# raphiniert-com/volume_renderer

Measured on AMD Instinct MI355X. Metric: Mrays/s + achieved HBM GB/s, 1024³ vol @ 1920×1080 HG-shaded, 1/2/4/8 GPU, higher is better.
Workload: dtype f32; 1 GPU; V_shell(1024) fp32 1024^3, 1920x1080, HG 2 lights (example1.m), on-the-fly gradient, rotate(125,25,0) f=3 dist=6 thr=0.9; lights=2, gradient=compute, parallelism=image-column partition x1 (block 16), depth_lanes=2, frames=serial, one HIP stream

## Files before the change

### volume_renderer_amd/csrc/vr_capi.hip

```cpp
#include <hip/hip_runtime.h>

#include <algorithm>
#include <chrono>
#include <cmath>
#include <cstdio>
#include <cstdlib>
#include <cstring>
#include <memory>
#include <mutex>
#include <map>
#include <set>
#include <array>
#include <sstream>
#include <string>
#include <queue>
#include <vector>

#include "../../include/vrhip.h"
#include "vr_device.h"
#include "vr_resources.h"

#ifndef VR_WITH_K8
#define VR_WITH_K8 0
#endif
// ... 661 lines not shown
  F.mode = P.num_lights == 0 ? 0 : (g_tex.grad_method == G_LOOKUP ? 2 : 1);
  F.ab_alias = same_tex(P.ab, P.em);
  const bool em_grid = P.em.p && !P.em.one;
  if (F.mode == 1)
    F.share = em_grid && same_tex(P.gem, P.em);
  else if (F.mode == 2)
    F.share = em_grid && P.gx.p && P.gy.p && P.gz.p && !P.gx.one && same_dims(P.gx, P.em) &&
              same_dims(P.gy, P.em) && same_dims(P.gz, P.em);
  P.re_is_em = same_tex(P.re, P.em) && P.em.p != nullptr;
  {
    drift_bound(F, nullptr);
    for (int i = 0; i < 3; ++i) {
      const float n = i == 0 ? P.em.fnx : (i == 1 ? P.em.fny : P.em.fnz);
      P.tap_off[i] = (float)((F.mode == 1 ? (double)P.gstep[i] * P.bscale[i] * n : 0.0) + 0.0625);
    }
    P.tap_half = half_texel_taps(P, F.mode, P.em.fnz);
    P.cube_hs[0] = P.tap_half ? P.em.fnx * 0.5f : 0.f;
    P.cube_hs[1] = P.tap_half ? P.em.fny * 0.5f : 0.f;
    P.cube_hs[2] = P.tap_half ? P.em.fnz * 0.5f : 0.f;
  }
  {
    const BufPtr &rb = g_tex.bind[g_tex.idx_re];
    const BufPtr &lb = g_tex.bind[T_LIGHT];
    bool ok = tame(rb) && tame(lb) && std::isfinite(P.fr) && std::fabs(P.fr) < 1e3f;
    double bound = 1.0;
    for (int i = 0; i < 3; ++i) {
      ok = ok && std::isfinite(P.color[i]) && std::fabs(P.color[i]) < 1e3f;
      bound = std::max(bound, (double)std::fabs(P.color[i]));
    }
    double lmax = 0.0;
    for (const auto &L : g_tex.lights) {
      for (float c : {L.cr, L.cg, L.cb}) {
        ok = ok && std::isfinite(c);
        lmax = std::max(lmax, (double)std::fabs(c));
      }
    }
    const double rmax = (rb && rb->ptr) ? rb->maxabs : 0.0, lutmax = (lb && lb->ptr) ? lb->maxabs : 0.0;
    ok = ok && (double)std::fabs(P.fr) * rmax * lutmax * lmax * bound * (double)(g_tex.lights.size() + 1) < 1e36;
    P.skip_empty = ok ? 1 : 0;
    if (const char *ev = test_env("VR_NO_EMPTY_SKIP"))
      if (ev[0] == '1') P.skip_empty = 0;
  }
  {
    const BufPtr &eb = g_tex.bind[g_tex.idx_em], &ab = g_tex.bind[g_tex.idx_ab];
    auto vmax = [](const BufPtr &b) { return (b && b->ptr) ? (b->nonfinite ? INFINITY : (double)b->maxabs) : 0.0; };
    const double xa = std::fabs((double)P.fa) * vmax(ab) * (double)P.tstep;
    const double xe = std::fabs((double)P.fe) * vmax(eb) * (double)P.tstep;
    P.small_x = (std::isfinite(xa) && xa < 0x1p-7 * 0.999) ? 1 : 0;
    P.eds_finite = (std::isfinite(xe) && xe < 1e38) ? 1 : 0;
    if (diag_flag("VR_NO_RANGE_FLAGS")) P.small_x = P.eds_finite = 0;
  }
  {
    const bool re_ok = P.re_is_em || (P.re.p && P.re.one);
    const bool lut_ok = g_tex.lights.empty() || (P.lut.p && P.lut.small && !P.lut.one && P.lut.zp);
    const bool step_ok = std::isfinite(P.tstep) && P.tstep > 0.f;
    P.tame = (P.skip_empty && P.eds_finite && P.small_x && re_ok && lut_ok && step_ok && !diag_flag("VR_NO_TAME")) ? 1
                                                                                                            : 0;
    P.re_mask = P.re_is_em ? 0xffffffffu : 0u;
  }
  F.big = is_big(P.em) || is_big(P.ab) || is_big(P.re) || is_big(P.gem) || is_big(P.gx) || is_big(P.gy) ||
          is_big(P.gz) || test_flag("VR_FORCE_BIG");
  if (F.mode == 2 && P.gx.p &&
      vr::interleave3_entries(P.gx.px, P.gx.pxy / P.gx.px, (uint32_t)P.gx.nz + 2u) > 0xFFFFFFFFull)
    F.big = true;
  if (is_big(P.lut)) return fail(VR_ERR_UNSUPPORTED, "illumination volume larger than 2^32 voxels");
  bool finite = std::isfinite(P.tstep) && P.tstep > 0.f;
  for (int i = 0; i < 3; ++i) finite = finite && std::isfinite(P.bmin[i]) && std::isfinite(P.bscale[i]);
  const double diag = std::sqrt(4.0 * ((double)bmax[0] * bmax[0] + (double)bmax[1] * bmax[1] +
                                       (double)bmax[2] * bmax[2]));
  const double cap = 2.0 * diag / (double)P.tstep + 64.0;
  P.max_steps = (finite && cap < 2.0e9) ? (int32_t)cap : 2000000000;
  F.degenerate = !finite;
  return VR_OK;
}

void upload_lights(vr_context *h, const vr_render_args *a) {
  if (a->num_lights < 0 || !a->illumination) return;
  const size_t n = (size_t)a->num_lights;
  g_tex.lights.resize(n);
  for (size_t l = 0; l < n; ++l) {
    const vr_light &L = a->lights[l];
    g_tex.lights[l] = vr::DevLight{L.position[2], L.position[1], L.position[0], L.color[0], L.color[1],
                                   L.color[2]};
  }
  h->vol[T_LIGHT] = make_rec(a->illumination);
  sync_volume_if_changed(h, T_LIGHT, T_LIGHT);
}

using LaunchRec = vr_host::LaunchRec<BufPtr>;
void wait_ready(const BufPtr &b, hipStream_t s) {
  if (b && !vr_host::done(b->ready)) VR_HIP(hipStreamWaitEvent(s, b->ready->e, 0));
}
void bind_reads(LaunchRec &L) {
  for (const BufPtr &b : g_tex.bind)
    if (b) {
      wait_ready(b, L.stream);
      L.reads.push_back(b);
    }
  for (const auto &kv : g_tex.gvec)
    if (kv.second.buf && kv.first == L.device) {
      wait_ready(kv.second.buf, L.stream);
      L.reads.push_back(kv.second.buf);
    }
}
void stage_frame(LaunchRec &L, vr::RenderParams &P, const std::vector<vr::DevLight> &lights) {
  const void *d = nullptr;
  VR_HIP(L.stage(lights.data(), lights.size() * sizeof(vr::DevLight), &d));
// ... 1977 lines not shown
```

### volume_renderer_amd/csrc/vr_march.hip

```cpp
#include <hip/hip_runtime.h>
#include <stdint.h>
#include <math.h>
#include <stdlib.h>
#include <algorithm>
#include <type_traits>

#ifndef VR_MARCH_K
#define VR_MARCH_K 1
#endif
#ifndef VR_MERGED_BOUNDS
#define VR_MERGED_BOUNDS 1
#endif
#ifndef VR_WHOLE_BOX
#define VR_WHOLE_BOX 1
#endif
#ifndef VR_CHECK_WHOLE
#define VR_CHECK_WHOLE 0
#endif
#ifndef VR_LIGHTS_HOIST
#define VR_LIGHTS_HOIST 1
#endif
#ifndef VR_REFL_HOIST
#define VR_REFL_HOIST 1
#endif
// ... 282 lines not shown
#undef iny
#undef inz
}

__device__ __forceinline__ void composite(const RenderParams &P, Ray &R, float r, float gg, float b, float alpha,
                                          float thr, int cap) {
  const float om = 1.f - R.sa;
  R.sr = fmaf(om, r, R.sr);
  R.sg = fmaf(om, gg, R.sg);
  R.sb = fmaf(om, b, R.sb);
  R.sa = fmaf(om, alpha, R.sa);
  ++R.nsteps;
  if (R.sa > thr || R.nsteps >= cap) {
    R.alive = false;
  } else {
    R.t += P.tstep;
    if (R.t > R.tfar) R.alive = false;
    else R.pos = mk(R.pos.x + R.step.x, R.pos.y + R.step.y, R.pos.z + R.step.z);
  }
}

#ifndef VR_GROUP_ANY_DPP
#define VR_GROUP_ANY_DPP 1
#endif
template <int K>
__device__ __forceinline__ bool group_any(bool b) {
  if constexpr ((K == 2 || K == 4) && VR_GROUP_ANY_DPP) {
    int v = b ? 1 : 0;
    v |= __builtin_amdgcn_mov_dpp(v, 0xB1, 0xf, 0xf, true);
    if constexpr (K == 4) v |= __builtin_amdgcn_mov_dpp(v, 0x4E, 0xf, 0xf, true);
    return v != 0;
  } else {
    const uint64_t m = __ballot(b);
    const int base = (int)(__lane_id() & ~(uint32_t)(K - 1));
    return ((m >> base) & ((1ull << K) - 1)) != 0ull;
  }
}

template <int K, int I = 0>
__device__ __forceinline__ int group_max_i(int v, int acc) {
  if constexpr (K == 1 || I == K) {
    return acc;
  } else {
    return group_max_i<K, I + 1>(v, max(acc, __float_as_int(group_lane<K, I>(__int_as_float(v)))));
  }
}

#ifndef VR_ZERO_FILL
#define VR_ZERO_FILL 1
#endif
template <int K, int I, bool ZF = false>
__device__ __forceinline__ void composite_group(const RenderParams &P, Ray &R, float exf, float r, float gg, float b,
                                                float alpha, float thr) {
  if constexpr (I < K) {
    const float ri = group_lane<K, I>(r), gi = group_lane<K, I>(gg), bi = group_lane<K, I>(b),
                ai = group_lane<K, I>(alpha);
    if ((ZF || group_lane<K, I>(exf) != 0.f) && R.alive) {
      const float om = 1.f - R.sa;
      R.sr = fmaf(om, ri, R.sr);
      R.sg = fmaf(om, gi, R.sg);
      R.sb = fmaf(om, bi, R.sb);
      R.sa = fmaf(om, ai, R.sa);
      if (R.sa > thr) R.alive = false;
    }
    composite_group<K, I + 1, ZF>(P, R, exf, r, gg, b, alpha, thr);
  }
}

template <int K, int MODE, bool AB_ALIAS, bool COUNT, bool SHARE2, bool BIG, bool NANCHK, int CAP, bool SLAB = false,
          int NL = 0>
__device__ __forceinline__ void march(const RenderParams &P, float *L, int lane, Ray &R, ChunkStats &C,
                                      uint32_t kk = 0, KParams kp = nullptr, uint32_t gw = 0) {
  static_assert(!COUNT || K == 1 || VR_COUNT_K, "the counter variant is built for K = 1 only (VR_COUNT_K: all K)");
  static_assert(!SLAB || (!COUNT && BIG), "slab mode: no counters, 64-bit addressing");
  const int cap = P.max_steps;
  const float thr = P.thr;
  const float sbz = P.bmin[2], ssz = P.bscale[2];
  auto beyond = [&](float zn) { return R.step.z >= 0.f ? zn >= P.slab_z1 : zn < P.slab_z0; };
  const DevTex &E = P.em;
  const int sub = lane & (K - 1);
  if constexpr (K > 1) {
    R.mine = R.alive;
    leap(P, sub, R.mine, R.nsteps, R.t, R.tfar, R.pos, R.step, cap);
    R.alive = group_any<K>(R.mine);
  }

  int s0 = VR_CHUNK;
  constexpr bool PROBE = VR_PROBE && !NANCHK && AB_ALIAS && !SLAB;
  int ps = VR_PROBE_MIN;
  float rv = 0.f;
  if constexpr (!NANCHK && VR_REFL_HOIST) {
    if (P.tame && P.re.p) rv = voxel0(P.re.p);
    asm volatile("" : "+v"(rv));
  }
  DevLight pre2[2];
  const DevLight *pre = nullptr;
  if constexpr (!NANCHK && VR_LIGHTS_HOIST && MODE != 0 && K > 1 && AB_ALIAS && SHARE2 && !BIG && !SLAB && !COUNT) {
    const bool two = NL == 2 || (NL == 0 && P.num_lights >= 2);
    for (int j = 0; j < 2; ++j) {
      pre2[j] = (two || (NL == 1 && j == 0)) ? light_at(P, j) : DevLight{0.f, 0.f, 0.f, 0.f, 0.f, 0.f};
      asm volatile("" : "+v"(pre2[j].px), "+v"(pre2[j].py), "+v"(pre2[j].pz), "+v"(pre2[j].cr), "+v"(pre2[j].cg),
                   "+v"(pre2[j].cb));
    }
    if (two || NL == 1) pre = pre2;
  }
  auto leap_run = [&](int n) __attribute__((always_inline)) {
    if constexpr (K == 1) {
// ... 110 lines not shown
    if (staged) {
      const bool nonzero = stage_box<BIG>(L, E, B, lane);
      empty = AB_ALIAS && P.skip_empty && !partial && !nonzero && (!SLAB || inside);
    }
    __builtin_amdgcn_wave_barrier();
    if (COUNT) ++(staged && !partial ? (empty ? C.leap : C.staged) : C.fall);
    const bool whole = __builtin_amdgcn_readfirstlane((!NANCHK && !SLAB && staged && !partial && !edge) ? 1 : 0) != 0;

    if (empty) {
      if (!parked_any) leap_run(S);
      else if (__float_as_int(R.t) >= 0) leap_run(S);
      unpark();
      if (PROBE && ps < 0) ps = VR_PROBE_MIN;
      continue;
    }
    if (PROBE) ps = (VR_PROBE_LANES && VR_REPROBE_PARTIAL && partial) ? (int)VR_PROBE_MIN : -1;

    if constexpr (K == 1) {
      for (int k = 0; k < S && R.alive; ++k) {
        if (SLAB && !inside) {
          const float zn = (R.pos.z - sbz) * ssz;
          if (!(zn >= P.slab_z0 && zn < P.slab_z1)) {
            if (beyond(zn)) {
              store_resume(P, kk, R.t, R.pos, R.nsteps);
              R.alive = false;
              R.past = true;
            } else {
              ++R.nsteps;
              if (R.nsteps >= P.max_steps) {
                R.alive = false;
              } else {
                R.t += P.tstep;
                if (R.t > R.tfar) R.alive = false;
                else R.pos = mk(R.pos.x + R.step.x, R.pos.y + R.step.y, R.pos.z + R.step.z);
              }
            }
            continue;
          }
        }
        float r, gg, b, alpha;
        bool shaded;
        sample_at<MODE, AB_ALIAS, SHARE2, BIG, NANCHK, NL>(P, L, B, staged, whole, R.pos, R.o, r, gg, b, alpha, shaded,
                                                       rv, pre);
        if (COUNT) {
          ++C.iter;
          C.lit += (MODE != 0 && __any(shaded)) ? 1u : 0u;
          R.nlit += shaded ? 1 : 0;
        }
        composite(P, R, r, gg, b, alpha, thr, cap);
      }
    } else {
      auto samples = [&](auto wc) {
      constexpr bool WC = decltype(wc)::value;
      for (int k = 0; k < S && R.alive; k += K) {
        float r = 0.f, gg = 0.f, b = 0.f, alpha = 0.f;
        bool ex = R.mine, take = R.mine;
        if (SLAB && !inside) {
          const float zn = (R.pos.z - sbz) * ssz;
          if (ex && beyond(zn)) ex = false;
          take = ex && zn >= P.slab_z0 && zn < P.slab_z1;
        }
        bool shaded = false;
        if (take) {
          sample_at<MODE, AB_ALIAS, SHARE2, BIG, NANCHK, NL>(P, L, B, staged, WC || (!VR_WHOLE_SPLIT && whole), R.pos,
                                                         R.o, r, gg, b, alpha, shaded, rv, pre);
        }
        if (COUNT) {
          ++C.iter;
          C.lit += (MODE != 0 && __any(shaded)) ? 1u : 0u;
        }
        composite_group<K, 0, VR_ZERO_FILL && !NANCHK && !SLAB>(P, R, ex ? 1.f : 0.f, r, gg, b, alpha, thr);
        if (SLAB && !inside) {
          if (R.alive && group_any<K>(R.mine && !ex)) {
            float t = R.t;
            f3 p = R.pos;
            int32_t n = R.nsteps;
            first_of_group<K>((R.mine && !ex) ? 1.f : 0.f, R.t, R.pos, R.nsteps, t, p, n);
            if (sub == 0) store_resume(P, kk, t, p, n);
            R.alive = false;
            R.past = true;
          }
        }
        if constexpr (!NANCHK && !SLAB)
          advance_k<K>(P, R.mine, R.nsteps, R.t, R.tfar, R.pos, R.step, cap);
        else
          advance(P, K, R.mine, R.nsteps, R.t, R.tfar, R.pos, R.step, cap);
        R.alive = R.alive && group_any<K>(R.mine);
      }
      };
      if constexpr (VR_WHOLE_SPLIT && !NANCHK && !SLAB && VR_MARCH_FAST && MODE == 1 && SHARE2) {
        if (whole) samples(std::true_type{});
        else samples(std::false_type{});
      } else {
        samples(std::false_type{});
      }
    }
    unpark();
    __builtin_amdgcn_wave_barrier();
  }
}

__device__ __forceinline__ bool finite3(const f3 &v) {
  return fabsf(v.x) <= 3.4e38f && fabsf(v.y) <= 3.4e38f && fabsf(v.z) <= 3.4e38f;
}

#ifndef VR_MARCH_MIN_EU
#define VR_MARCH_MIN_EU 5
// ... 42 lines not shown
    wgo += P.block_rot;
    if (wgo >= gridDim.x) wgo -= gridDim.x;
  }
  if (ORDERED && blockIdx.x < P.prio_blocks) __builtin_amdgcn_s_setprio(2);
  int view, lc, y;
  if constexpr (PAIRED) {
    constexpr int TH2 = TS::TH / 2, HR = (64 / K) / 2;
    const int tile = (int)wgo * VR_WG_WAVES + wave;
    const int nbx = (P.part_cols + P.pair_shift + 2 * TS::TW - 1) / (2 * TS::TW);
    const int blk = tile >> 2, quad = tile & 3;
    const int ray = lane >> TS::LK, rr = ray & (HR - 1);
    view = ray >= HR ? 0 : 1;
    const int xv = (blk % nbx) * (2 * TS::TW) + (quad & 1) * TS::TW + rr / TH2;
    y = (blk / nbx) * (2 * TH2) + (quad >> 1) * TH2 + rr % TH2;
    lc = view ? xv - P.pair_shift : xv;
  } else {
    view = (P.views > 1 && wgo >= P.view_blocks) ? 1 : 0;
    const uint32_t wg = view ? wgo - P.view_blocks : wgo;
    const int tile = (int)wg * VR_WG_WAVES + wave;
    const int nbx = (P.part_cols + 2 * TS::TW - 1) / (2 * TS::TW);
    const int blk = tile >> 2, quad = tile & 3;
    const int ray = lane >> TS::LK;
    lc = (blk % nbx) * (2 * TS::TW) + (quad & 1) * TS::TW + (ray / TS::TH);
    y = (blk / nbx) * (2 * TS::TH) + (quad >> 1) * TS::TH + (ray % TS::TH);
  }
  float *const out = view ? P.out2 : P.out;
  const bool active = (!PAIRED || lc >= 0) && (lc < P.part_cols) && (y < P.height);
  Ray R;
  R.o = mk(0.f, 0.f, 0.f);
  R.pos = R.o;
  R.step = R.o;
  R.t = 0.f;
  R.tfar = -1.f;
  R.sr = R.sg = R.sb = R.sa = 0.f;
  R.nsteps = R.nlit = 0;
  R.alive = false;
  ChunkStats C{0, 0, 0, 0, 0, 0, 0};
  if (active) {
    const int blk = lc / P.block_cols, within = lc - blk * P.block_cols;
    const int x = (P.part + blk * P.num_parts) * P.block_cols + within;
    f3 d;
    float tnear;
    R.alive = ray_setup(P, x, y, R.o, d, tnear, R.tfar, view);
    R.pos = mk(fmaf(d.x, tnear, R.o.x), fmaf(d.y, tnear, R.o.y), fmaf(d.z, tnear, R.o.z));
    R.step = mk(d.x * P.tstep, d.y * P.tstep, d.z * P.tstep);
    R.t = tnear;
  }
  if (P.tame && __all(!R.alive || (finite3(R.pos) && finite3(R.step))))
    march<K, MODE, AB_ALIAS, COUNT, SHARE2, BIG, false, CAP, false, NL>(
        P, L, lane, R, C, 0u, (KParams)__builtin_amdgcn_kernarg_segment_ptr(), wgo * VR_WG_WAVES + (uint32_t)wave);
  else
    march<K, MODE, AB_ALIAS, COUNT, SHARE2, BIG, true, CAP>(P, L, lane, R, C);

  if (active && (lane & (K - 1)) == 0) {
    const size_t plane = (size_t)P.plane_cols * (size_t)P.height;
    const size_t kk = (size_t)lc * (size_t)P.height + (size_t)y;
    out[kk] = R.sr;
    out[kk + plane] = R.sg;
    out[kk + 2 * plane] = R.sb;
  }
  if (TIMED) {
    __syncthreads();
    if (threadIdx.x == 0) {
      const uint64_t d = __builtin_amdgcn_s_memrealtime() - clk0;
      P.wg_cost[wgo] = d > 0xffffffffull ? 0xffffffffu : (uint32_t)d;
      if (P.wg_start) P.wg_start[wgo] = (uint32_t)clk0;
    }
  }
  if (COUNT) {
    unsigned long long s = K == 1 ? (unsigned long long)R.nsteps : 0ull, l = K == 1 ? (unsigned long long)R.nlit : 0ull;
#pragma unroll
    for (int off = 32; off > 0; off >>= 1) {
      s += __shfl_xor(s, off, 64);
      l += __shfl_xor(l, off, 64);
    }
    if (lane == 0 && s) atomicAdd(P.steps, s);
    if (lane == 0 && l) atomicAdd(P.steps + 1, l);
    if (lane == 0) {
      atomicAdd(P.steps + 2, (unsigned long long)C.staged);
      atomicAdd(P.steps + 3, (unsigned long long)C.leap);
      atomicAdd(P.steps + 4, (unsigned long long)C.fall);
      atomicAdd(P.steps + 5, (unsigned long long)C.iter);
      atomicAdd(P.steps + 6, (unsigned long long)C.lit);
      atomicAdd(P.steps + 7, (unsigned long long)C.probe);
      atomicAdd(P.steps + 44, (unsigned long long)C.probe_fail);
    }
  }
}

template <int K>
__global__ __launch_bounds__(64 * VR_WG_WAVES) void preleap_kernel(const RenderParams P) {
  using TS = TileShape<K>;
  const int lane = threadIdx.x & 63, wave = threadIdx.x >> 6;
  const uint32_t wgo = blockIdx.x;
  const uint32_t gw = wgo * VR_WG_WAVES + (uint32_t)wave;
  const int view = (P.views > 1 && wgo >= P.view_blocks) ? 1 : 0;
  const uint32_t wg = view ? wgo - P.view_blocks : wgo;
  const int tile = (int)wg * VR_WG_WAVES + wave;
  const int nbx = (P.part_cols + 2 * TS::TW - 1) / (2 * TS::TW);
  const int blk = tile >> 2, quad = tile & 3;
  const int ray = lane >> TS::LK;
  const int lc = (blk % nbx) * (2 * TS::TW) + (quad & 1) * TS::TW + (ray / TS::TH);
  const int y = (blk / nbx) * (2 * TS::TH) + (quad >> 1) * TS::TH + (ray % TS::TH);
  const bool active = lc < P.part_cols && y < P.height;
  Ray R;
  R.pos = mk(0.f, 0.f, 0.f);
  R.step = R.pos;
// ... 422 lines not shown
```

### volume_renderer_amd/csrc/vr_sampling.h

```cpp
#pragma once
#include <hip/hip_runtime.h>
#include <stdint.h>
#include <math.h>

#include "vr_device.h"

namespace vr {

#define VR_PI ((float)3.14159265358979323846f)

struct f3 {
  float x, y, z;
};
__device__ __forceinline__ f3 mk(float x, float y, float z) { return f3{x, y, z}; }
__device__ __forceinline__ float dot3(f3 a, f3 b) { return fmaf(a.z, b.z, fmaf(a.y, b.y, a.x * b.x)); }

typedef float f2a4 __attribute__((ext_vector_type(2), aligned(4)));
typedef float f4a8 __attribute__((ext_vector_type(4), aligned(8)));

struct Ax {
  int i;
  float w;
};
__device__ __forceinline__ float weight8(float xb, float fl) {
  return fmaf(rintf(xb * 256.f), 1.f / 256.f, -fl);
}
template <bool NANCHK = true>
__device__ __forceinline__ Ax axis(float c, int n, float fn) {
  if (NANCHK) c = (c != c) ? 0.f : c;
  const float xb = c * fn - 0.5f;
  const float fl = floorf(xb);
  const float w = weight8(xb, fl);
  (void)n;
  return Ax{(int)__builtin_amdgcn_fmed3f(fl, -1.f, fn - 1.f), w};
}

template <bool NANCHK = true>
__device__ __forceinline__ Ax axis_raw(float c, float fn) {
  if (NANCHK) c = (c != c) ? 0.f : c;
  const float xb = c * fn - 0.5f;
  const float fl = floorf(xb);
  const float w = weight8(xb, fl);
  return Ax{(int)fl, w};
}
__device__ __forceinline__ Ax clamp_ax(const Ax &a, int n) { return Ax{min(max(a.i, -1), n - 1), a.w}; }

struct AxS {
  int i;
  float w;
  bool hi;
};
template <bool NANCHK = true>
__device__ __forceinline__ AxS axis_raw_s(float c, float fn) {
  if (NANCHK) c = (c != c) ? 0.f : c;
  const float xb = c * fn - 0.5f;
  const float fl = floorf(xb);
  const float r = xb - fl;
  const float w = rintf(r * 256.f) * (1.f / 256.f);
  return AxS{(int)fl, w, r >= 0.5f};
}
template <bool NANCHK = true>
__device__ __forceinline__ AxS axis_cube_s(float p, float hs) {
  float a = p + 1.f;
  if (NANCHK) a = (a != a) ? 0.f : a;
  const float xb = fmaf(a, hs, -0.5f);
  const float fl = floorf(xb);
  const float r = xb - fl;
  const float w = rintf(r * 256.f) * (1.f / 256.f);
  return AxS{(int)fl, w, r >= 0.5f};
}

__device__ __forceinline__ void half_taps(const AxS &a, Ax &plus, Ax &minus) {
  const int ip = a.i + (a.hi ? 1 : 0);
  const float wt = a.w + (a.hi ? -0.5f : 0.5f);
  plus = Ax{ip, wt};
  minus = Ax{ip - 1, wt};
}

__device__ __forceinline__ float sqrt_cr(float x) {
  const uint32_t u = __float_as_uint(x);
  if (__builtin_expect(__all(u - 1u >= 0x0f7fffffu), 1)) {
    const float s = __builtin_amdgcn_sqrtf(x);
    const float sm = __uint_as_float(__float_as_uint(s) - 1u), sp = __uint_as_float(__float_as_uint(s) + 1u);
    const float rm = fmaf(-sm, s, x), rp = fmaf(-sp, s, x);
    const float r = (rm <= 0.f) ? sm : s;
    return (rp > 0.f) ? sp : r;
  }
  return sqrtf(x);
}

__device__ __forceinline__ float sqrt_fast(float x) {
  const float s = __builtin_amdgcn_sqrtf(x);
  const float sm = __uint_as_float(__float_as_uint(s) - 1u), sp = __uint_as_float(__float_as_uint(s) + 1u);
  const float rm = fmaf(-sm, s, x), rp = fmaf(-sp, s, x);
  const float r = (rm <= 0.f) ? sm : s;
  return (rp > 0.f) ? sp : r;
}
template <int N>
__device__ __forceinline__ void sqrt_cr_n(const float (&x)[N], float (&out)[N]) {
  bool ok = true;
#pragma unroll
  for (int i = 0; i < N; ++i) ok = ok && (__float_as_uint(x[i]) - 1u >= 0x0f7fffffu);
  if (__builtin_expect(__all(ok), 1)) {
#pragma unroll
    for (int i = 0; i < N; ++i) out[i] = sqrt_fast(x[i]);
  } else {
#pragma unroll
    for (int i = 0; i < N; ++i) out[i] = sqrtf(x[i]);
  }
}

__device__ __forceinline__ float lerp(float a, float b, float w) { return fmaf(w, b - a, a); }

template <bool BIG>
__device__ __forceinline__ float fetch(const DevTex &t, const Ax &ax, const Ax &ay, const Ax &az) {
  const float *b;
  if (BIG) {
    const uint64_t o = ((uint64_t)(az.i + 1) * t.pxy + (uint64_t)(ay.i + 1) * t.px) + (uint64_t)(ax.i + 1);
    b = t.p + o;
  } else {
    const uint32_t o = ((uint32_t)(az.i + 1) * t.pxy + (uint32_t)(ay.i + 1) * t.px) + (uint32_t)(ax.i + 1);
    b = t.p + o;
  }
  const f2a4 r00 = *reinterpret_cast<const f2a4 *>(b);
  const f2a4 r10 = *reinterpret_cast<const f2a4 *>(b + t.px);
  const f2a4 r01 = *reinterpret_cast<const f2a4 *>(b + t.pxy);
  const f2a4 r11 = *reinterpret_cast<const f2a4 *>(b + t.pxy + t.px);
  const float c00 = lerp(r00.x, r00.y, ax.w), c10 = lerp(r10.x, r10.y, ax.w);
  const float c01 = lerp(r01.x, r01.y, ax.w), c11 = lerp(r11.x, r11.y, ax.w);
  const float c0 = lerp(c00, c10, ay.w), c1 = lerp(c01, c11, ay.w);
  return lerp(c0, c1, az.w);
}

struct AxF {
  float fl;
  float w;
};

template <bool FMA = false>
__device__ __forceinline__ AxF axis_lut(float c, float fn) {
  c = __builtin_amdgcn_fmed3f(c, 0.f, 1.f);
  const float xb = FMA ? fmaf(c, fn, -0.5f) : c * fn - 0.5f;
  const float fl = floorf(xb);
  return AxF{fl, weight8(xb, fl)};
}

__device__ __forceinline__ float fetch_small(const DevTex &t, const AxF &ax, const AxF &ay, const AxF &az) {
  const uint32_t o = (uint32_t)fmaf(az.fl, t.fpxy4, fmaf(ay.fl, t.fpx4, fmaf(ax.fl, 4.f, t.fbase4)));
  const uint32_t px4 = t.px * 4u, pxy4 = t.pxy * 4u;
  const char *b = reinterpret_cast<const char *>(t.p);
  const f2a4 r00 = *reinterpret_cast<const f2a4 *>(b + o);
  const f2a4 r10 = *reinterpret_cast<const f2a4 *>(b + (o + px4));
  const f2a4 r01 = *reinterpret_cast<const f2a4 *>(b + (o + pxy4));
  const f2a4 r11 = *reinterpret_cast<const f2a4 *>(b + (o + pxy4 + px4));
  const float c00 = lerp(r00.x, r00.y, ax.w), c10 = lerp(r10.x, r10.y, ax.w);
  const float c01 = lerp(r01.x, r01.y, ax.w), c11 = lerp(r11.x, r11.y, ax.w);
  const float c0 = lerp(c00, c10, ay.w), c1 = lerp(c01, c11, ay.w);
  return lerp(c0, c1, az.w);
}
__device__ __forceinline__ void fetch_small2(const DevTex &t, const AxF &ax, const AxF &ay0, const AxF &az0,
                                             const AxF &ay1, const AxF &az1, float &v0, float &v1) {
  const float ox = fmaf(ax.fl, 4.f, t.fbase4);
  const uint32_t o0 = (uint32_t)fmaf(az0.fl, t.fpxy4, fmaf(ay0.fl, t.fpx4, ox));
  const uint32_t o1 = (uint32_t)fmaf(az1.fl, t.fpxy4, fmaf(ay1.fl, t.fpx4, ox));
  const uint32_t px4 = t.px * 4u, pxy4 = t.pxy * 4u;
  const char *b = reinterpret_cast<const char *>(t.p);
  const f2a4 a00 = *reinterpret_cast<const f2a4 *>(b + o0);
  const f2a4 a10 = *reinterpret_cast<const f2a4 *>(b + (o0 + px4));
  const f2a4 a01 = *reinterpret_cast<const f2a4 *>(b + (o0 + pxy4));
  const f2a4 a11 = *reinterpret_cast<const f2a4 *>(b + (o0 + pxy4 + px4));
  const f2a4 b00 = *reinterpret_cast<const f2a4 *>(b + o1);
  const f2a4 b10 = *reinterpret_cast<const f2a4 *>(b + (o1 + px4));
  const f2a4 b01 = *reinterpret_cast<const f2a4 *>(b + (o1 + pxy4));
  const f2a4 b11 = *reinterpret_cast<const f2a4 *>(b + (o1 + pxy4 + px4));
  {
    const float c00 = lerp(a00.x, a00.y, ax.w), c10 = lerp(a10.x, a10.y, ax.w);
    const float c01 = lerp(a01.x, a01.y, ax.w), c11 = lerp(a11.x, a11.y, ax.w);
    v0 = lerp(lerp(c00, c10, ay0.w), lerp(c01, c11, ay0.w), az0.w);
  }
  {
    const float c00 = lerp(b00.x, b00.y, ax.w), c10 = lerp(b10.x, b10.y, ax.w);
    const float c01 = lerp(b01.x, b01.y, ax.w), c11 = lerp(b11.x, b11.y, ax.w);
    v1 = lerp(lerp(c00, c10, ay1.w), lerp(c01, c11, ay1.w), az1.w);
  }
}
#ifndef VR_LUT_ZPAIR
#define VR_LUT_ZPAIR 1
#endif
__device__ __forceinline__ float lerp_zrows(const f4a8 &r0, const f4a8 &r1, const AxF &ax, const AxF &ay,
                                            const AxF &az) {
  const float c00 = lerp(r0.x, r0.z, ax.w), c10 = lerp(r1.x, r1.z, ax.w);
  const float c01 = lerp(r0.y, r0.w, ax.w), c11 = lerp(r1.y, r1.w, ax.w);
  const float c0 = lerp(c00, c10, ay.w), c1 = lerp(c01, c11, ay.w);
  return lerp(c0, c1, az.w);
}
__device__ __forceinline__ float fetch_small_z(const DevTex &t, const AxF &ax, const AxF &ay, const AxF &az) {
  const uint32_t o = (uint32_t)fmaf(az.fl, t.fpxy4, fmaf(ay.fl, t.fpx4, fmaf(ax.fl, 4.f, t.fbase4)));
// ... 320 lines not shown

__device__ __forceinline__ DevLight light_at(const RenderParams &P, int i) {
  typedef const __attribute__((address_space(4))) DevLight *cptr;
  const cptr q = (cptr)P.lights + i;
  return DevLight{q->px, q->py, q->pz, q->cr, q->cg, q->cb};
}
__device__ __forceinline__ float voxel0(const float *p) {
  typedef const __attribute__((address_space(4))) float *cptr;
  return ((cptr)p)[0];
}

template <bool TAME, bool XN, bool XG, bool NEED, int NL = 0>
__device__ __forceinline__ void shade_fast(const RenderParams &P, const f3 g, const f3 pos, const f3 o,
                                          const float refl, float &ir, float &ig, float &ib, bool &need,
                                          const DevLight *pre = nullptr) {
  static_assert(NL == 0 || ((NL == 1 || NL == 2) && TAME), "specialised for hoisted lights only");
  const int nl = NL ? NL : P.num_lights;
  float ginv;
  if constexpr (XN) ginv = rcp_sqrt_cr(dot3(g, g));
  else if (VR_FAST_NXQ) ginv = __builtin_amdgcn_rcpf(__builtin_amdgcn_sqrtf(dot3(g, g)));
  else ginv = __builtin_amdgcn_rsqf(dot3(g, g));
  const f3 n = mk(-(g.x * ginv), -(g.y * ginv), -(g.z * ginv));
  const f3 li = mk(o.x - pos.x, o.y - pos.y, o.z - pos.z);
  const float dli = dot3(li, n);
  const f3 lip = mk(fmaf(-dli, n.x, li.x), fmaf(-dli, n.y, li.y), fmaf(-dli, n.z, li.z));
#if VR_FAST_NLEN
  const float rn = 1.f;
#else
  const float rn = rsq_c(dot3(n, n));
#endif
  const float lip2 = dot3(lip, lip), li2 = dot3(li, li);
  const float rlip = XG ? sqrt_cr(lip2) : (VR_FAST_GXQ ? __builtin_amdgcn_sqrtf(lip2) : rsq_c(lip2));
  auto gamma_q = [&](const f3 &lo, const f3 &lop) {
    const float lop2 = dot3(lop, lop);
    float q;
    if constexpr (XG) q = div_acos_arg(dot3(lip, lop), rlip * sqrt_cr(lop2));
    else if (VR_FAST_GXQ) q = div_short(dot3(lip, lop), rlip * __builtin_amdgcn_sqrtf(lop2));
    else q = dot3(lip, lop) * (rlip * rsq_c(lop2));
    if constexpr (NEED) need = need || fabsf(q) > VR_HYB_TG || lop2 < VR_HYB_TA * dot3(lo, lo);
    if constexpr (VR_FAST_HYBQ == 2 && !XG && !NEED) {
      const float aq = fabsf(q);
      if (__builtin_expect(aq > VR_HYB_TG && aq < VR_HYB_TU, 0)) q = dot3(lip, lop) / (sqrtf(lip2) * sqrtf(lop2));
    } else if constexpr (VR_FAST_HYBQ == 1 && !XG && !NEED) {
      const bool nd = fabsf(q) > VR_HYB_TG;
      if (__builtin_expect(__any(nd), 0)) {
        const float qx = div_acos_arg(dot3(lip, lop), sqrt_cr(lip2) * sqrt_cr(lop2));
        if (nd) q = qx;
      }
    }
    return q;
  };
  if constexpr (NEED) need = lip2 < VR_HYB_TA * li2;
  const float alpha_n = acospi_f(dot3(n, li) * (rn * rsq_c(li2)));
  const AxF la = axis_lut<true>(alpha_n, P.lut.fnx);
  int i = 0;
  if (TAME || (P.lut.p != nullptr && P.lut.small && !P.lut.one)) {
    for (; i + 1 < nl; i += 2) {
      const DevLight L0 = NL == 2 ? pre[0] : ((pre && i == 0) ? pre[0] : light_at(P, i));
      const DevLight L1 = NL == 2 ? pre[1] : ((pre && i == 0) ? pre[1] : light_at(P, i + 1));
      const f3 lo0 = mk(L0.px - pos.x, L0.py - pos.y, L0.pz - pos.z);
      const f3 lo1 = mk(L1.px - pos.x, L1.py - pos.y, L1.pz - pos.z);
      const float dlo0 = dot3(lo0, n), dlo1 = dot3(lo1, n);
      const f3 lop0 = mk(fmaf(-dlo0, n.x, lo0.x), fmaf(-dlo0, n.y, lo0.y), fmaf(-dlo0, n.z, lo0.z));
      const f3 lop1 = mk(fmaf(-dlo1, n.x, lo1.x), fmaf(-dlo1, n.y, lo1.y), fmaf(-dlo1, n.z, lo1.z));
      const float beta0 = acospi_f(dlo0 * (rn * rsq_c(dot3(lo0, lo0))));
      const float gamma0 = acospi_f(gamma_q(lo0, lop0));
      const float beta1 = acospi_f(dlo1 * (rn * rsq_c(dot3(lo1, lo1))));
      const float gamma1 = acospi_f(gamma_q(lo1, lop1));
      float light0, light1;
#if VR_ABLATE & 1
      light0 = beta0 + gamma0 + la.w;
      light1 = beta1 + gamma1 + la.w;
#else
      if (TAME && VR_LUT_ZPAIR)
        fetch_small2_z(P.lut, la, axis_lut<true>(beta0, P.lut.fny), axis_lut<true>(gamma0, P.lut.fnz),
                       axis_lut<true>(beta1, P.lut.fny), axis_lut<true>(gamma1, P.lut.fnz), light0, light1);
      else
        fetch_small2(P.lut, la, axis_lut<true>(beta0, P.lut.fny), axis_lut<true>(gamma0, P.lut.fnz),
                     axis_lut<true>(beta1, P.lut.fny), axis_lut<true>(gamma1, P.lut.fnz), light0, light1);
#endif
      const float rl0 = refl * light0;
      ir = fmaf(rl0 * L0.cr, P.color[0], ir);
      ig = fmaf(rl0 * L0.cg, P.color[1], ig);
      ib = fmaf(rl0 * L0.cb, P.color[2], ib);
      const float rl1 = refl * light1;
      ir = fmaf(rl1 * L1.cr, P.color[0], ir);
      ig = fmaf(rl1 * L1.cg, P.color[1], ig);
      ib = fmaf(rl1 * L1.cb, P.color[2], ib);
    }
  }
  if constexpr (!TAME) for (; i + 1 < nl; i += 2) {
    const DevLight L0 = light_at(P, i), L1 = light_at(P, i + 1);
    const f3 lo0 = mk(L0.px - pos.x, L0.py - pos.y, L0.pz - pos.z);
    const f3 lo1 = mk(L1.px - pos.x, L1.py - pos.y, L1.pz - pos.z);
    const float dlo0 = dot3(lo0, n), dlo1 = dot3(lo1, n);
    const f3 lop0 = mk(fmaf(-dlo0, n.x, lo0.x), fmaf(-dlo0, n.y, lo0.y), fmaf(-dlo0, n.z, lo0.z));
    const f3 lop1 = mk(fmaf(-dlo1, n.x, lo1.x), fmaf(-dlo1, n.y, lo1.y), fmaf(-dlo1, n.z, lo1.z));
    const float beta0 = acospi_f(dlo0 * (rn * rsq_c(dot3(lo0, lo0))));
    const float gamma0 = acospi_f(gamma_q(lo0, lop0));
    const float beta1 = acospi_f(dlo1 * (rn * rsq_c(dot3(lo1, lo1))));
    const float gamma1 = acospi_f(gamma_q(lo1, lop1));
    const float light0 = lut_light<true>(P.lut, la, beta0, gamma0);
    const float light1 = lut_light<true>(P.lut, la, beta1, gamma1);
    const float rl0 = refl * light0;
    ir = fmaf(rl0 * L0.cr, P.color[0], ir);
    ig = fmaf(rl0 * L0.cg, P.color[1], ig);
    ib = fmaf(rl0 * L0.cb, P.color[2], ib);
    const float rl1 = refl * light1;
    ir = fmaf(rl1 * L1.cr, P.color[0], ir);
    ig = fmaf(rl1 * L1.cg, P.color[1], ig);
    ib = fmaf(rl1 * L1.cb, P.color[2], ib);
  }
  if (i < nl) {
    const DevLight L = NL == 1 ? pre[0] : light_at(P, i);
    const f3 lo = mk(L.px - pos.x, L.py - pos.y, L.pz - pos.z);
    const float dlo = dot3(lo, n);
    const f3 lop = mk(fmaf(-dlo, n.x, lo.x), fmaf(-dlo, n.y, lo.y), fmaf(-dlo, n.z, lo.z));
    const float beta = acospi_f(dlo * (rn * rsq_c(dot3(lo, lo))));
    const float gamma = acospi_f(gamma_q(lo, lop));
    const float rl = refl * (TAME ? (VR_LUT_ZPAIR ? fetch_small_z(P.lut, la, axis_lut<true>(beta, P.lut.fny),
                                                                 axis_lut<true>(gamma, P.lut.fnz))
                                                  : fetch_small(P.lut, la, axis_lut<true>(beta, P.lut.fny),
                                                                axis_lut<true>(gamma, P.lut.fnz)))
                                  : lut_light<true>(P.lut, la, beta, gamma));
    ir = fmaf(rl * L.cr, P.color[0], ir);
    ig = fmaf(rl * L.cg, P.color[1], ig);
    ib = fmaf(rl * L.cb, P.color[2], ib);
  }
}

template <bool FAST, bool TAME = false, int NL = 0>
__device__ __forceinline__ void shade_lights(const RenderParams &P, const f3 g, const f3 pos, const f3 o,
                                             const float refl, float &ir, float &ig, float &ib,
                                             const DevLight *pre = nullptr) {
#if !VR_FAST_COS
  if constexpr (FAST) {
    const float ginv = 1.f / sqrt_cr(dot3(g, g));
    const f3 n = mk(-(g.x * ginv), -(g.y * ginv), -(g.z * ginv));
    const f3 li = mk(o.x - pos.x, o.y - pos.y, o.z - pos.z);
    const float dli = dot3(li, n);
    const f3 lip = mk(fmaf(-dli, n.x, li.x), fmaf(-dli, n.y, li.y), fmaf(-dli, n.z, li.z));
    float sq_in[3] = {dot3(n, n), dot3(li, li), dot3(lip, lip)}, sq[3];
    sqrt_cr_n<3>(sq_in, sq);
    const float nlen = sq[0], liplen = sq[2];
    float alpha_n;
    {
      const float num[1] = {dot3(n, li)}, den[1] = {nlen * sq[1]};
      float q[1];
      div_acos_n<1>(num, den, q);
      alpha_n = acospi_q(q[0]);
    }
    const AxF la = axis_lut<true>(alpha_n, P.lut.fnx);
    for (int i = 0; i < P.num_lights; ++i) {
      const DevLight L = light_at(P, i);
      const f3 lo = mk(L.px - pos.x, L.py - pos.y, L.pz - pos.z);
      const float dlo = dot3(lo, n);
      const f3 lop = mk(fmaf(-dlo, n.x, lo.x), fmaf(-dlo, n.y, lo.y), fmaf(-dlo, n.z, lo.z));
      float li_in[2] = {dot3(lo, lo), dot3(lop, lop)}, ln[2];
      sqrt_cr_n<2>(li_in, ln);
      const float num[2] = {dot3(n, lo), dot3(lip, lop)}, den[2] = {nlen * ln[0], liplen * ln[1]};
      float q[2];
      div_acos_n<2>(num, den, q);
      const float rl = refl * lut_light<true>(P.lut, la, acospi_q(q[0]), acospi_q(q[1]));
      ir = fmaf(rl * L.cr, P.color[0], ir);
      ig = fmaf(rl * L.cg, P.color[1], ig);
      ib = fmaf(rl * L.cb, P.color[2], ib);
    }
  } else
#endif
  if constexpr (FAST) {
#if VR_FAST_HYBRID
    bool need = false;
    const float ir0 = ir, ig0 = ig, ib0 = ib;
    shade_fast<TAME, false, false, true>(P, g, pos, o, refl, ir, ig, ib, need);
    if (__any(need)) {
      float er = ir0, eg = ig0, eb = ib0;
// ... 102 lines not shown
```

Measured before the change: 83.33 Mrays/s.

## Use DPP fmac compositing, wave-uniform march loop, and magic-number 8-bit weight rounding

For two depth lanes with zero-fill, compositing now uses inline-asm v_fmac_f32_dpp with quad_perm in place of separate lane shuffles followed by FMAs. The sample loop bound is made wave-uniform via readfirstlane and exits when no lane in the wave is alive, instead of testing each lane's alive flag in the loop condition. The 8-bit interpolation weight rounding replaces rintf(r*256)/256 with an add/subtract of a magic constant on the tame and no-NaN-check paths, and the tame path now requires LUT dimensions of at most 8192 so this rounding stays exact. The output-write lane test uses __lane_id(). The inline asm relies on a hand-placed s_nop for the DPP hazard and adds a dependency on the exact register and lane layout.

```diff
diff --git a/volume_renderer_amd/csrc/vr_capi.hip b/volume_renderer_amd/csrc/vr_capi.hip
--- a/volume_renderer_amd/csrc/vr_capi.hip
+++ b/volume_renderer_amd/csrc/vr_capi.hip
@@ -737,7 +737,8 @@
   }
   {
     const bool re_ok = P.re_is_em || (P.re.p && P.re.one);
-    const bool lut_ok = g_tex.lights.empty() || (P.lut.p && P.lut.small && !P.lut.one && P.lut.zp);
+    const bool lut_ok = g_tex.lights.empty() || (P.lut.p && P.lut.small && !P.lut.one && P.lut.zp &&
+                                                 std::max(P.lut.nx, std::max(P.lut.ny, P.lut.nz)) <= 8192);
     const bool step_ok = std::isfinite(P.tstep) && P.tstep > 0.f;
     P.tame = (P.skip_empty && P.eds_finite && P.small_x && re_ok && lut_ok && step_ok && !diag_flag("VR_NO_TAME")) ? 1
                                                                                                             : 0;
diff --git a/volume_renderer_amd/csrc/vr_march.hip b/volume_renderer_amd/csrc/vr_march.hip
--- a/volume_renderer_amd/csrc/vr_march.hip
+++ b/volume_renderer_amd/csrc/vr_march.hip
@@ -358,7 +358,29 @@
 template <int K, int I, bool ZF = false>
 __device__ __forceinline__ void composite_group(const RenderParams &P, Ray &R, float exf, float r, float gg, float b,
                                                 float alpha, float thr) {
-  if constexpr (I < K) {
+  if constexpr (K == 2 && ZF && I < K) {
+    if (R.alive) {
+      const float om = 1.f - R.sa;
+      if constexpr (I == 0)
+        asm("s_nop 1\n\t"
+            "v_fmac_f32_dpp %0, %4, %8 quad_perm:[0,0,2,2] row_mask:0xf bank_mask:0xf\n\t"
+            "v_fmac_f32_dpp %1, %5, %8 quad_perm:[0,0,2,2] row_mask:0xf bank_mask:0xf\n\t"
+            "v_fmac_f32_dpp %2, %6, %8 quad_perm:[0,0,2,2] row_mask:0xf bank_mask:0xf\n\t"
+            "v_fmac_f32_dpp %3, %7, %8 quad_perm:[0,0,2,2] row_mask:0xf bank_mask:0xf"
+            : "+v"(R.sr), "+v"(R.sg), "+v"(R.sb), "+v"(R.sa)
+            : "v"(r), "v"(gg), "v"(b), "v"(alpha), "v"(om));
+      else
+        asm("s_nop 1\n\t"
+            "v_fmac_f32_dpp %0, %4, %8 quad_perm:[1,1,3,3] row_mask:0xf bank_mask:0xf\n\t"
+            "v_fmac_f32_dpp %1, %5, %8 quad_perm:[1,1,3,3] row_mask:0xf bank_mask:0xf\n\t"
+            "v_fmac_f32_dpp %2, %6, %8 quad_perm:[1,1,3,3] row_mask:0xf bank_mask:0xf\n\t"
+            "v_fmac_f32_dpp %3, %7, %8 quad_perm:[1,1,3,3] row_mask:0xf bank_mask:0xf"
+            : "+v"(R.sr), "+v"(R.sg), "+v"(R.sb), "+v"(R.sa)
+            : "v"(r), "v"(gg), "v"(b), "v"(alpha), "v"(om));
+      if (R.sa > thr) R.alive = false;
+    }
+    composite_group<K, I + 1, ZF>(P, R, exf, r, gg, b, alpha, thr);
+  } else if constexpr (I < K) {
     const float ri = group_lane<K, I>(r), gi = group_lane<K, I>(gg), bi = group_lane<K, I>(b),
                 ai = group_lane<K, I>(alpha);
     if ((ZF || group_lane<K, I>(exf) != 0.f) && R.alive) {
@@ -575,7 +597,9 @@
     } else {
       auto samples = [&](auto wc) {
       constexpr bool WC = decltype(wc)::value;
-      for (int k = 0; k < S && R.alive; k += K) {
+      for (int k = 0, Su = __builtin_amdgcn_readfirstlane(S); k < Su; k += K) {
+        if (!__any(R.alive)) break;
+        if (!R.alive) continue;
         float r = 0.f, gg = 0.f, b = 0.f, alpha = 0.f;
         bool ex = R.mine, take = R.mine;
         if (SLAB && !inside) {
@@ -724,7 +748,7 @@
   else
     march<K, MODE, AB_ALIAS, COUNT, SHARE2, BIG, true, CAP>(P, L, lane, R, C);
 
-  if (active && (lane & (K - 1)) == 0) {
+  if (active && (__lane_id() & (K - 1)) == 0) {
     const size_t plane = (size_t)P.plane_cols * (size_t)P.height;
     const size_t kk = (size_t)lc * (size_t)P.height + (size_t)y;
     out[kk] = R.sr;
diff --git a/volume_renderer_amd/csrc/vr_sampling.h b/volume_renderer_amd/csrc/vr_sampling.h
--- a/volume_renderer_amd/csrc/vr_sampling.h
+++ b/volume_renderer_amd/csrc/vr_sampling.h
@@ -25,6 +25,9 @@
 __device__ __forceinline__ float weight8(float xb, float fl) {
   return fmaf(rintf(xb * 256.f), 1.f / 256.f, -fl);
 }
+#define VR_RN_MAGIC 49152.f
+__device__ __forceinline__ float frac8_rn(float r) { return (r + VR_RN_MAGIC) - VR_RN_MAGIC; }
+__device__ __forceinline__ float weight8_rn(float xb, float fl) { return ((xb + VR_RN_MAGIC) - VR_RN_MAGIC) - fl; }
 template <bool NANCHK = true>
 __device__ __forceinline__ Ax axis(float c, int n, float fn) {
   if (NANCHK) c = (c != c) ? 0.f : c;
@@ -56,7 +59,7 @@
   const float xb = c * fn - 0.5f;
   const float fl = floorf(xb);
   const float r = xb - fl;
-  const float w = rintf(r * 256.f) * (1.f / 256.f);
+  const float w = NANCHK ? rintf(r * 256.f) * (1.f / 256.f) : frac8_rn(r);
   return AxS{(int)fl, w, r >= 0.5f};
 }
 template <bool NANCHK = true>
@@ -66,7 +69,7 @@
   const float xb = fmaf(a, hs, -0.5f);
   const float fl = floorf(xb);
   const float r = xb - fl;
-  const float w = rintf(r * 256.f) * (1.f / 256.f);
+  const float w = NANCHK ? rintf(r * 256.f) * (1.f / 256.f) : frac8_rn(r);
   return AxS{(int)fl, w, r >= 0.5f};
 }
 
@@ -137,12 +140,12 @@
   float w;
 };
 
-template <bool FMA = false>
+template <bool FMA = false, bool RN8 = false>
 __device__ __forceinline__ AxF axis_lut(float c, float fn) {
   c = __builtin_amdgcn_fmed3f(c, 0.f, 1.f);
   const float xb = FMA ? fmaf(c, fn, -0.5f) : c * fn - 0.5f;
   const float fl = floorf(xb);
-  return AxF{fl, weight8(xb, fl)};
+  return AxF{fl, RN8 ? weight8_rn(xb, fl) : weight8(xb, fl)};
 }
 
 __device__ __forceinline__ float fetch_small(const DevTex &t, const AxF &ax, const AxF &ay, const AxF &az) {
@@ -569,7 +572,7 @@
   };
   if constexpr (NEED) need = lip2 < VR_HYB_TA * li2;
   const float alpha_n = acospi_f(dot3(n, li) * (rn * rsq_c(li2)));
-  const AxF la = axis_lut<true>(alpha_n, P.lut.fnx);
+  const AxF la = axis_lut<true, TAME>(alpha_n, P.lut.fnx);
   int i = 0;
   if (TAME || (P.lut.p != nullptr && P.lut.small && !P.lut.one)) {
     for (; i + 1 < nl; i += 2) {
@@ -590,11 +593,11 @@
       light1 = beta1 + gamma1 + la.w;
 #else
       if (TAME && VR_LUT_ZPAIR)
-        fetch_small2_z(P.lut, la, axis_lut<true>(beta0, P.lut.fny), axis_lut<true>(gamma0, P.lut.fnz),
-                       axis_lut<true>(beta1, P.lut.fny), axis_lut<true>(gamma1, P.lut.fnz), light0, light1);
+        fetch_small2_z(P.lut, la, axis_lut<true, TAME>(beta0, P.lut.fny), axis_lut<true, TAME>(gamma0, P.lut.fnz),
+                       axis_lut<true, TAME>(beta1, P.lut.fny), axis_lut<true, TAME>(gamma1, P.lut.fnz), light0, light1);
       else
-        fetch_small2(P.lut, la, axis_lut<true>(beta0, P.lut.fny), axis_lut<true>(gamma0, P.lut.fnz),
-                     axis_lut<true>(beta1, P.lut.fny), axis_lut<true>(gamma1, P.lut.fnz), light0, light1);
+        fetch_small2(P.lut, la, axis_lut<true, TAME>(beta0, P.lut.fny), axis_lut<true, TAME>(gamma0, P.lut.fnz),
+                     axis_lut<true, TAME>(beta1, P.lut.fny), axis_lut<true, TAME>(gamma1, P.lut.fnz), light0, light1);
 #endif
       const float rl0 = refl * light0;
       ir = fmaf(rl0 * L0.cr, P.color[0], ir);
@@ -635,10 +638,10 @@
     const f3 lop = mk(fmaf(-dlo, n.x, lo.x), fmaf(-dlo, n.y, lo.y), fmaf(-dlo, n.z, lo.z));
     const float beta = acospi_f(dlo * (rn * rsq_c(dot3(lo, lo))));
     const float gamma = acospi_f(gamma_q(lo, lop));
-    const float rl = refl * (TAME ? (VR_LUT_ZPAIR ? fetch_small_z(P.lut, la, axis_lut<true>(beta, P.lut.fny),
-                                                                 axis_lut<true>(gamma, P.lut.fnz))
-                                                  : fetch_small(P.lut, la, axis_lut<true>(beta, P.lut.fny),
-                                                                axis_lut<true>(gamma, P.lut.fnz)))
+    const float rl = refl * (TAME ? (VR_LUT_ZPAIR ? fetch_small_z(P.lut, la, axis_lut<true, TAME>(beta, P.lut.fny),
+                                                                 axis_lut<true, TAME>(gamma, P.lut.fnz))
+                                                  : fetch_small(P.lut, la, axis_lut<true, TAME>(beta, P.lut.fny),
+                                                                axis_lut<true, TAME>(gamma, P.lut.fnz)))
                                   : lut_light<true>(P.lut, la, beta, gamma));
     ir = fmaf(rl * L.cr, P.color[0], ir);
     ig = fmaf(rl * L.cg, P.color[1], ig);
```

Result: faster. 85.45 Mrays/s, median of 6 (+2.5%).
